# keychera/raytracing-clj

Measured on AMD Instinct MI355X. Metric: Mray-samples/sec at 1200×675×100spp depth50; achieved HBM GB/s vs peak, higher is better.
Workload: dtype fp32

## Files before the change

raytracing-clj_amd/csrc/trace.hip:

```cpp
#include "trace_kernel.h"
#include "first_hit.h"
#include "bvh_refit.h"
#include "dscene.h"

namespace rtclj {

__device__ __forceinline__ int cost_bucket(unsigned c) {
  if (c < 8) return static_cast<int>(c);
  const int e = 31 - __clz(c);
  return ((e - 2) << 3) | static_cast<int>((c >> (e - 3)) & 7u);
}
__global__ __launch_bounds__(1024) void order_kernel(unsigned* __restrict__ cost, int* __restrict__ order,
                                                     int n) {
  __shared__ int hist[256];
  __shared__ int cursor[256];
  __shared__ int scan[256];
  const int t = static_cast<int>(threadIdx.x);
  if (t < 256) hist[t] = 0;
  __syncthreads();
  for (int i = t; i < n; i += 1024) atomicAdd(&hist[cost_bucket(cost[i])], 1);
  __syncthreads();
  if (t < 256) scan[t] = hist[255 - t];
  __syncthreads();
  for (int off = 1; off < 256; off <<= 1) {
// ... 115 lines not shown
  for (int p = p0; p < p1; ++p) sum += fin(p);
  __syncthreads();
  s_part[tid] = sum;
  __syncthreads();
  if (tid == 0) {
    int run = 0;
    for (int i = 0; i < 1024; ++i) {
      const int v = s_part[i];
      s_part[i] = run;
      run += v;
    }
    s_left = run;
  }
  __syncthreads();
  int base = s_part[tid];
  for (int p = p0; p < p1; ++p) {
    const int sp = fin(p);
    const int tile = order[p];
    for (int k = 0; k < sp; ++k) units[base + k] = make_int2(tile, k | (sp << 8));
    base += sp;
  }
  for (int u = s_left + tid; u < U; u += 1024) units[u] = make_int2(-1, 0);
}

#ifdef RTCLJ_DIAG
constexpr bool kDiag = true;
#else
constexpr bool kDiag = false;
#endif
static_assert(policy::kTile == kTile && policy::kPoolPx == kPoolPx && policy::kXBytes == kXBytes,
              "variant_policy.h: the kernels' shapes");
constexpr bool traits_agree() {
  for (const policy::Traits& t : policy::kTraits) {
    if (t.build == policy::BUILD_NONE) continue;
    const int walk = t.scan == SCAN_BVHS ? policy::WALK_SORTED : is_bvh_scan(t.scan) ? policy::WALK_BVH : policy::WALK_NONE;
    if (t.walk != walk || t.tree != scan_tree(t.scan) || t.compact != is_compact_scan(t.scan) ||
        t.entry_bytes != stack_entry_bytes(t.scan) || policy::variant_rows(t) != (t.th ? t.th : tile_rows(t.scan)) ||
        (walk == policy::WALK_SORTED && t.threads != kSortThreads))
      return false;
  }
  return true;
}
static_assert(traits_agree(), "variant_policy.h: a row's columns against its scan's traits");

const void* trace_kernel_w16();
static const policy::Traits& variant_traits(int v) { return policy::traits(v, kDiag); }
static const void* variant_fn(int v) {
  switch (v) {
    case policy::kDefault: return RT_K(SRC_LDS, SCAN_BVHQ, false);
    case policy::kScan: return RT_K(SRC_SCALAR, SCAN_GROUP4, false);
    case policy::kGlobal: return RT_K(SRC_SCALAR, SCAN_BVH, false);
    case policy::kFull4: return RT_K(SRC_LDS, SCAN_BVHQ, false);
    case policy::kLeaf8: return RT_KW(SRC_LDS, SCAN_BVHO, false, 8);
    case policy::kCompact: return RT_K(SRC_LDS, SCAN_BVHQ7, false);
    case policy::kCompactW8: return RT_KW(SRC_LDS, SCAN_BVHQ7, false, 8);
    case policy::kCompactW16: return trace_kernel_w16();
    case policy::kCompactTh4: return RT_KWT(SRC_LDS, SCAN_BVHQ7, false, 4, 4);
  }
#ifdef RTCLJ_DIAG
  return diag_kernel(v);
#else
  return nullptr;
#endif
}
static const void* variant_sweep(int v) { return v == policy::kCompact ? RT_KSW(SRC_LDS, SCAN_BVHQ7, 4, 0) : nullptr; }

static std::atomic<int> g_variant{0};
static std::atomic<int> g_schedule{0};
static const bool g_bvh_sah = bvh_sah_default();
#ifdef RTCLJ_DIAG
static const bool g_timeline = [] {
  const char* e = std::getenv("RTCLJ_TIMELINE");
  return e && std::atoi(e) != 0;
}();
#endif
constexpr int kDbg = 32;
constexpr int kDbgDevices = 64;
static std::mutex g_dbg_mu;
static unsigned long long* g_dbg[kDbgDevices] = {};
static unsigned long long* g_dbgw[kDbgDevices] = {};

int selected_variant() { return g_variant.load(); }
bool diag_build() { return kDiag; }

}

using namespace rtclj;

hipError_t rtclj::fill_words(void* p, uint32_t word, size_t n, hipStream_t stream) {
  if (n == 0) return hipSuccess;
  const size_t blocks = std::min<size_t>((n + 255) / 256, 2048);
  return enqueue(fill_kernel, dim3(static_cast<unsigned>(blocks)), dim3(256), 0, stream, static_cast<uint32_t*>(p), word, n);
}

namespace rtclj {
int fill_async(void* p, int byte_value, size_t bytes, void* stream) {
  if (bytes % 4 != 0) return hipErrorInvalidValue;
  return fill_words(p, static_cast<uint32_t>(byte_value & 0xff) * 0x01010101u, bytes / 4, static_cast<hipStream_t>(stream));
}

int quantize_launch(const float* d_lin, uint8_t* d_out, size_t n, void* stream) {
  if (n == 0) return hipSuccess;
  const size_t blocks = std::min<size_t>((n + 255) / 256, 4096);
  return enqueue(quantize_kernel, dim3(static_cast<unsigned>(blocks)), dim3(256), 0, static_cast<hipStream_t>(stream), d_lin,
                 d_out, n, quantize_table());
}
}

static std::atomic<uint64_t> g_scene_uid{0};
uint64_t rtclj::scene_uid(const rt_dscene* ds) { return ds ? ds->uid : 0; }
// ... 738 lines not shown
```

raytracing-clj_amd/csrc/trace_kernel.h:

```cpp
#pragma once
#include <hip/hip_runtime.h>

#include <algorithm>
#include <chrono>
#include <atomic>
#include <climits>
#include <cstdlib>
#include <cmath>
#include <cstdint>
#include <cstring>
#include <mutex>
#include <string>
#include <thread>
#include <type_traits>
#include <vector>

#include "bvh.h"
#include "bvh_pad.h"
#include "fp_rn.h"
#include "rt_internal.h"

namespace rtclj {

struct alignas(16) KArgs {
  const float4* geo;
  const struct Pair* geo2;
  const float4* sph;
  const float4* mat;
  const int* kind;
  float* out;
  unsigned long long* counters;
  unsigned long long* dbg;
  unsigned long long* dbgw;
  float cam[18];
  int defocus;
  int n;
  int n_pad;
  int width;
  int rows_out;
  int row_begin, row_tile, tile_first, tile_step;
  const float4* bvh_blob;
  int bvh_blob_f4;
  int bvh_off_pairs;
  int bvh_off_pidx;
  int big_pair0;
  int n_big_leaves;
  int bvh_stack;
  float bvh_c[3], bvh_r;
  float bvh_c0;
  const int* tile_order;
  unsigned* tile_cost;
  unsigned long long* part;
  int tiles_x;
  int n_whole, split;
  const int2* unit_tab;
  uint64_t rt_magic;
  int spp, sample_begin, max_depth;
  int realm;
  int sampler;
  uint32_t key;
  unsigned long long* word;
  unsigned* done;
  unsigned long long* sum;
  int* owner;
  unsigned long long* stealc;
  int n_owner;
  int n_units;
  int share_from;
  int steal_min;
  int batch_max;
  int lds_batch_max;
  unsigned epoch;
  int compact;
// ... 158 lines not shown
  asm volatile("" : "+s"(p));
  return p;
}

enum { SRC_LDS = 1, SRC_SCALAR = 2 };
enum { SCAN_SIMPLE = 0, SCAN_GROUP4 = 1, SCAN_PK4 = 2, SCAN_BVH = 3, SCAN_BVHWW = 4, SCAN_BVHQ = 5, SCAN_BVHO = 6,
       SCAN_BVHS = 7 ,
       SCAN_BVHQ7 = 8  };
constexpr bool is_bvh_scan(int scan) { return (scan >= SCAN_BVH && scan <= SCAN_BVHO) || scan == SCAN_BVHQ7; }
constexpr bool is_q(int scan) { return scan == SCAN_BVHQ || scan == SCAN_BVHQ7; }
constexpr int leaf_pairs(int scan) { return scan == SCAN_BVHO ? 4 : is_q(scan) ? 2 : 1; }
constexpr int scan_tree(int scan) { return scan == SCAN_BVHO ? 2 : (is_q(scan) || scan == SCAN_BVHS) ? 1 : 0; }
constexpr bool is_compact_scan(int scan) { return scan == SCAN_BVHQ7; }
constexpr int stack_entry_bytes(int scan) { return (scan == SCAN_BVHO || scan == SCAN_BVHQ7) ? 1 : 2; }

typedef float f2 __attribute__((ext_vector_type(2)));
typedef const char __attribute__((address_space(3)))* LdsC;
typedef const f2 __attribute__((address_space(3)))* LdsF2;
typedef float f4v __attribute__((ext_vector_type(4)));
typedef const f4v __attribute__((address_space(3)))* LdsF4;
typedef const long long __attribute__((address_space(3)))* LdsI64;
__device__ __forceinline__ unsigned lds_addr(const void* p) { return static_cast<unsigned>((uintptr_t)(LdsC)p); }
struct alignas(16) Pair {
  f2 x, y, z, w;
};
__device__ __forceinline__ f2 fma2(f2 a, f2 b, f2 c) { return __builtin_elementwise_fma(a, b, c); }
__device__ __forceinline__ float fma3(float a, float b, float c) {
  float r;
  asm("v_fma_f32 %0, %1, %2, %3" : "=v"(r) : "v"(a), "v"(b), "v"(c));
  return r;
}
__device__ __forceinline__ f2 bc_lo(f2 v) { return __builtin_shufflevector(v, v, 0, 0); }
__device__ __forceinline__ f2 bc_hi(f2 v) { return __builtin_shufflevector(v, v, 1, 1); }

struct alignas(16) KNode {
  f2 x[3], y[3], z[3];
  int c0, c1;
};
static_assert(sizeof(KNode) == 80, "KNode layout");

constexpr int kTile = 8;
constexpr int kLeafRecBytes = 80;
constexpr int kPoolPx = kTile * kTile;
constexpr int tile_rows(int scan) { return scan == SCAN_BVHS ? 16 : kTile; }

constexpr int min_waves(int scan, bool stats, int nw = 4) {
  return stats ? 1 : scan == SCAN_BVHQ ? 6 : scan == SCAN_BVHQ7 ? (nw == 16 ? 8 : 7) : scan == SCAN_BVHO ? 3 : 1;
}

template <int SRC, int SCAN, class F>
__device__ void diag_scan(const struct KArgs& a, const float4* s_geo, float ox, float oy, float oz, float ux,
                          float uy, float uz, F&& consider);

template <int SRC, int SCAN, bool STATS = false, int NW = 4, int THT = 0, bool SWEEP = false>
__global__ __launch_bounds__(64 * NW, min_waves(SCAN, STATS, NW)) void trace_kernel(const KArgs a) {
  constexpr int NT = 64 * NW;
  __shared__ int s_pool_next;
  __shared__ int s_cnt;
  __shared__ int s_join;
  __shared__ int s_unit[2];
  __shared__ unsigned long long s_best;
  __shared__ unsigned long long s_segs;
  __shared__ int s_last;
  __shared__ int s_mb_post[NW], s_mb_take[NW], s_alive, s_mb_avail;
  __shared__ int s_mb_lim[NW];
  constexpr int TH = THT ? THT : tile_rows(SCAN);
  constexpr int NPX = kTile * TH;
  using AccT = std::conditional_t<SCAN == SCAN_BVHQ7, unsigned, unsigned long long>;
  __shared__ AccT s_acc[NPX * 3];
  uint64_t st_iter = 0, st_lanes = 0, st_sph = 0, st_blk = 0, st_blk_lanes = 0;
  uint64_t st_trav = 0, st_trav_lanes = 0;
  uint64_t st_leafw = 0, st_consw = 0;
  uint64_t st_ball = 0, st_disk = 0;
  uint64_t st_fl = 0;
  uint64_t st_fresh = 0, st_fresh_lanes = 0;
  uint64_t st_diel = 0, st_diel_lanes = 0;
  uint64_t st_lm = 0, st_lm_lanes = 0;
  uint64_t st_sums = 0, st_refill = 0, st_claim = 0, st_drain = 0;
  uint64_t st_c_cam = 0, st_c_scan = 0, st_c_shade = 0, st_c_acc = 0, st_ts = 0;
  uint64_t st_t0 = 0;
  if (STATS || a.tile_cost || a.dbgw) st_t0 = __builtin_amdgcn_s_memrealtime();
  extern __shared__ __attribute__((aligned(16))) float4 s_geo[];
  const int n = a.n;
  const int lane = threadIdx.x & 63;
  const int unit = static_cast<int>(blockIdx.x);
  const KArgsP ka = kargs_opaque();
  const bool own = SWEEP || unit < ka->n_units;
  int xpool = 0;
  if constexpr (SWEEP) {
    xpool = static_cast<int>(__hip_atomic_load(&ka->xq_n[0], __ATOMIC_RELAXED, __HIP_MEMORY_SCOPE_AGENT));
    if (unit * NT >= xpool) return;
  }
  auto tile_pool = [&](KArgsP kp, int t) {
    const int ty = t / kp->tiles_x, tx = t - ty * kp->tiles_x;
    const int w = max(0, min(kTile, kp->width - tx * kTile)), h = max(0, min(TH, kp->rows_out - ty * TH));
    return kp->spp > 0 && kp->max_depth > 0 ? w * h * kp->spp : 0;
  };
  if (!own) {
    if (!ka->word) return;
    if (threadIdx.x == 0) {
      s_best = 0ull;
      s_unit[0] = -1;
    }
    __syncthreads();
    const int M = ka->n_owner;
    const int w0 = static_cast<int>(mix32(static_cast<uint32_t>(unit)) % static_cast<uint32_t>(M));
    unsigned long long key = 0;
// ... 120 lines not shown
  };
  const float cx = a.cam[0], cy = a.cam[1], cz = a.cam[2];

  const int k0 = split ? static_cast<int>(static_cast<int64_t>(split_ix) * ka->spp / nsplit) : 0;
  const int cnt = split ? static_cast<int>(static_cast<int64_t>(split_ix + 1) * ka->spp / nsplit) - k0 : ka->spp;
  const int pool = SWEEP ? xpool : (cnt > 0 && ka->max_depth > 0) ? npx * cnt : 0;
  const uint32_t mag_vw = vw > 0 ? 0xffffffffu / static_cast<uint32_t>(vw) + 1u : 0u;
  const uint32_t mag16_vw = vw > 0 ? (65536u + static_cast<uint32_t>(vw) - 1u) / static_cast<uint32_t>(vw) : 0u;
  const uint64_t npx_magic = npx > 1 ? ~0ull / static_cast<uint64_t>(npx) + 1ull : 0ull;
  const bool shared_tile = !SWEEP && ka->word && !split && (!own || (pool > 512 && unit >= ka->share_from));
  unsigned long long* const src = shared_tile ? ka->word + tile : nullptr;
  const int kc_batch_max = ka->batch_max > 0 ? ka->batch_max : min(1024, max(kShareBatch, (pool / 48) & ~63));
  if (threadIdx.x == 0) {
    if (own && shared_tile) {
      __hip_atomic_exchange(&ka->word[tile], (static_cast<unsigned long long>(ka->epoch) << 48) | static_cast<unsigned long long>(NT),
                            __ATOMIC_RELAXED, __HIP_MEMORY_SCOPE_AGENT);
      __hip_atomic_exchange(&ka->owner[unit % ka->n_owner], tile, __ATOMIC_RELAXED, __HIP_MEMORY_SCOPE_AGENT);
      s_cnt = NT;
    }
    s_join = own ? 0 : 1;
    s_segs = 0ull;
    s_pool_next = NT;
    s_alive = NW;
    s_mb_avail = 0;
  }
  if (threadIdx.x < NW) {
    s_mb_post[threadIdx.x] = 0;
    s_mb_take[threadIdx.x] = 0;
    s_mb_lim[threadIdx.x] = ka->compact > 0 ? ka->compact : -1;
  }
  if (threadIdx.x < NPX * 3) s_acc[threadIdx.x] = 0;
  constexpr bool kPixelTable = is_q(SCAN) && !SWEEP;
  constexpr bool kCompactPx = SCAN == SCAN_BVHQ7;
  __shared__ std::conditional_t<kCompactPx, uint32_t, float4> s_px[kPixelTable ? NPX : 1];
  __shared__ float s_prow[kCompactPx ? TH : 1];
  if constexpr (kPixelTable) {
    const int t = static_cast<int>(threadIdx.x);
    if (t < npx) {
      const int qy = vw == 1 ? t : static_cast<int>(__umulhi(static_cast<uint32_t>(t), mag_vw));
      const int px = qx0 + (t - qy * vw);
      const int gy = image_row(qy0 + qy);
      if constexpr (kCompactPx) {
        s_px[t] = pixel_key(px, gy);
        if (px == qx0) s_prow[qy] = static_cast<float>(gy);
      } else {
        s_px[t] = make_float4(__uint_as_float(pixel_key(px, gy)), static_cast<float>(px), static_cast<float>(gy), 0.0f);
      }
    }
  }
  __shared__ uint32_t s_carry[kCompactPx ? NPX * 3 / 4 : 1];
  if constexpr (kCompactPx) {
    if (threadIdx.x < NPX * 3 / 4) s_carry[threadIdx.x] = 0u;
  }
  __syncthreads();
  int wb = 0, we = 0;
  int j = first + static_cast<int>(threadIdx.x), q = 0, k = 0;
  bool active = j < pool;
  if (!active) j = -2;

  uint32_t st = 0;
  float ox = 0, oy = 0, oz = 0, dx = 0, dy = 0, dz = 0;
  float tr = 1, tg = 1, tb = 1;
  int rem = 0;
  int last = -1;
  bool fresh = true;


  constexpr bool kCompact = is_bvh_scan(SCAN);
  const int wv = static_cast<int>(threadIdx.x >> 6);
  auto mb_word = [&](int d, int f, int p, int P) -> uint32_t* {
    constexpr int SZ = static_cast<int>(sizeof(StackT));
    constexpr int W = 16 * SZ;
    const int i = f * P + p;
    return reinterpret_cast<uint32_t*>(reinterpret_cast<char*>(s_stack) + (i / W) * NT * SZ + d * 64 * SZ +
                                       (i % W) * 4);
  };
  auto lds_load = [](int* p) { return __hip_atomic_load(p, __ATOMIC_ACQUIRE, __HIP_MEMORY_SCOPE_WORKGROUP); };
  auto compact_step = [&]() {
    RT_MARK("compact_step");
    const int wu = static_cast<int>(__builtin_amdgcn_readfirstlane(threadIdx.x >> 6));
    const int P = kargs_opaque()->mb_paths;
    const int leader = static_cast<int>(__builtin_amdgcn_readfirstlane(lane));
    const uint64_t live = __ballot(active);
    const int left = static_cast<int>(__popcll(live));
    bool out = false;
    bool post = false;
    if constexpr (!SWEEP) {
      uint4* const xq = kargs_opaque()->xq;
      if (xq) {
        if (left > 0) {
          int base = 0;
          if (lane == leader) base = static_cast<int>(atomicAdd(&kargs_opaque()->xq_n[0], static_cast<unsigned>(left)));
          base = __builtin_amdgcn_readlane(base, leader);
          const int rank = static_cast<int>(__builtin_amdgcn_mbcnt_hi(static_cast<uint32_t>(live >> 32),
                                                                      __builtin_amdgcn_mbcnt_lo(static_cast<uint32_t>(live), 0u)));
          if (active) {
            const int qy = static_cast<int>(__umul24(static_cast<uint32_t>(q), mag16_vw) >> 16);
            const int pix = (qy0 + qy) * kargs_opaque()->width + qx0 + (q - qy * vw);
            uint4* r = xq + 4 * static_cast<size_t>(base + rank);
            r[0] = make_uint4(__float_as_uint(ox), __float_as_uint(oy), __float_as_uint(oz), __float_as_uint(dx));
            r[1] = make_uint4(__float_as_uint(dy), __float_as_uint(dz), __float_as_uint(tr), __float_as_uint(tg));
            r[2] = make_uint4(__float_as_uint(tb), st, static_cast<uint32_t>(pix), static_cast<uint32_t>(rem));
            reinterpret_cast<uint32_t*>(r + 3)[0] = static_cast<uint32_t>(last);
          }
        }
        if (lane == leader) atomicAdd(&s_alive, -1);
        active = false;
// ... 36 lines not shown
          __hip_atomic_store(&s_mb_post[wu], 0, __ATOMIC_RELAXED, __HIP_MEMORY_SCOPE_WORKGROUP);
          atomicAdd(&s_mb_avail, -left);
        }
      }
      old = __builtin_amdgcn_readlane(old, leader);
      if (old > 1) {
        active = false;
        j = -2;
        return;
      }
      out = true;
    }
    uint64_t freem = ~live;
    bool took = false;
#pragma unroll 1
    for (int d = 0; d < NW && freem; ++d) {
      if (d == wu) continue;
      const int posted = sgpr(lds_load(&s_mb_post[d]));
      if (posted <= sgpr(lds_load(&s_mb_take[d]))) continue;
      const int want = static_cast<int>(__popcll(freem));
      int t0 = 0;
      if (lane == leader) t0 = atomicAdd(&s_mb_take[d], want);
      t0 = __builtin_amdgcn_readlane(t0, leader);
      const int got = min(want, posted - t0);
      if (got <= 0) continue;
      if (lane == leader) atomicAdd(&s_mb_avail, -got);
      const int rank = static_cast<int>(__builtin_amdgcn_mbcnt_hi(static_cast<uint32_t>(freem >> 32),
                                                                  __builtin_amdgcn_mbcnt_lo(static_cast<uint32_t>(freem), 0u)));
      const bool mine = ((freem >> lane) & 1ull) && rank < got;
      if (mine) {
        const int p = t0 + rank;
        ox = __uint_as_float(*mb_word(d, 0, p, P));
        oy = __uint_as_float(*mb_word(d, 1, p, P));
        oz = __uint_as_float(*mb_word(d, 2, p, P));
        dx = __uint_as_float(*mb_word(d, 3, p, P));
        dy = __uint_as_float(*mb_word(d, 4, p, P));
        dz = __uint_as_float(*mb_word(d, 5, p, P));
        tr = __uint_as_float(*mb_word(d, 6, p, P));
        tg = __uint_as_float(*mb_word(d, 7, p, P));
        tb = __uint_as_float(*mb_word(d, 8, p, P));
        st = *mb_word(d, 9, p, P);
        q = static_cast<int>(*mb_word(d, 10, p, P));
        rem = static_cast<int>(*mb_word(d, 11, p, P));
        last = static_cast<int>(*mb_word(d, 12, p, P));
        active = true;
        fresh = false;
        j = -1;
      }
      freem &= ~__ballot(mine);
      took = true;
    }
    if (out && (took || left > 0) && lane == leader) atomicAdd(&s_alive, 1);
  };
  auto iteration = [&]() {
    bool done = false;
    if constexpr (STATS) st_ts = stamp();
    if constexpr (STATS) {
      const uint64_t ex = __builtin_amdgcn_read_exec();
      if (lane == __ffsll(static_cast<long long>(ex)) - 1) {
        ++st_iter;
        st_lanes += __popcll(ex);
      }
    }
    RT_MARK("iteration");
    if (kCompact ? j >= 0 : fresh) {
      RT_MARK("camera");
      if constexpr (SWEEP) {
        const uint4* r = kargs_opaque()->xq + 4 * static_cast<size_t>(j);
        const uint4 r0 = r[0], r1 = r[1], r2 = r[2];
        const uint32_t r3 = reinterpret_cast<const uint32_t*>(r + 3)[0];
        ox = __uint_as_float(r0.x);
        oy = __uint_as_float(r0.y);
        oz = __uint_as_float(r0.z);
        dx = __uint_as_float(r0.w);
        dy = __uint_as_float(r1.x);
        dz = __uint_as_float(r1.y);
        tr = __uint_as_float(r1.z);
        tg = __uint_as_float(r1.w);
        tb = __uint_as_float(r2.x);
        st = r2.y;
        q = static_cast<int>(r2.z);
        rem = static_cast<int>(r2.w);
        last = static_cast<int>(r3);
        fresh = false;
        j = -1;
      } else {
      if constexpr (STATS) {
        const uint64_t ex = __builtin_amdgcn_read_exec();
        if (lane == __ffsll(static_cast<long long>(ex)) - 1) {
          ++st_fresh;
          st_fresh_lanes += __popcll(ex);
        }
      }
      k = div_magic(j, npx_magic);
      q = j - k * npx;
      uint32_t pk;
      float fpx, fgy;
      if constexpr (kPixelTable && kCompactPx) {
        pk = s_px[q];
        const int qy = static_cast<int>(__umul24(static_cast<uint32_t>(q), mag16_vw) >> 16);
        fpx = static_cast<float>(qx0 + (q - qy * vw));
        fgy = s_prow[qy];
      } else if constexpr (kPixelTable) {
        const float4 pt = s_px[q];
        pk = __float_as_uint(pt.x);
        fpx = pt.y;
        fgy = pt.z;
      } else {
        const int qy = vw == 1 ? q : static_cast<int>(__umulhi(static_cast<uint32_t>(q), mag_vw));
        const int px = qx0 + (q - qy * vw);
        const int gy = image_row(qy0 + qy);
        pk = pixel_key(px, gy);
        fpx = static_cast<float>(px);
        fgy = static_cast<float>(gy);
      }
      st = mix32(pk + static_cast<uint32_t>(a.sample_begin + k0 + k) * 0x9e3779b9u);
// ... 206 lines not shown
          if constexpr (STATS) {
            const uint64_t ex = __builtin_amdgcn_read_exec();
            if (lane == __ffsll(static_cast<long long>(ex)) - 1) ++st_consw;
          }
          const unsigned k = __builtin_ctz(m);
          m &= m - 1;
          float h = hh[0], d = dd[0];
          int s = ii[0];
#pragma unroll
          for (int j = 1; j < 2 * NP; ++j) {
            h = k == static_cast<unsigned>(8 * j) ? hh[j] : h;
            d = k == static_cast<unsigned>(8 * j) ? dd[j] : d;
            s = k == static_cast<unsigned>(8 * j) ? ii[j] : s;
          }
          consider_tie(h, d, s);
        }
        }
      };
      auto node_planes = [&](int node, float& tn0, float& tn1, float& tf0, float& tf1, int& c0, int& c1) {
        if constexpr (STATS) st_fl += 24;
        const unsigned nof = SCAN == SCAN_BVHQ    ? static_cast<unsigned>(node)
                             : SCAN == SCAN_BVHQ7 ? __umul24(static_cast<unsigned>(node), 80u) + lds_addr(nodes)
                                                  : __umul24(static_cast<unsigned>(node), 80u);
        f2 x0, x1, y0, y1, z0, z1;
        int2 ch;
        if constexpr (SRC == SRC_LDS && is_q(SCAN)) {
          const LdsF2 lx = (LdsF2)(uintptr_t)(nof + offx), ly = (LdsF2)(uintptr_t)(nof + offy),
                      lz = (LdsF2)(uintptr_t)(nof + offz);
          x0 = lx[0], x1 = lx[1], y0 = ly[0], y1 = ly[1], z0 = lz[0], z1 = lz[1];
          const long long c2 = *(LdsI64)(uintptr_t)(nof + 72);
          ch = make_int2(static_cast<int>(c2), static_cast<int>(c2 >> 32));
        } else {
          const char* nb = reinterpret_cast<const char*>(nodes) + nof;
          const f2* ax = reinterpret_cast<const f2*>(nb + offx);
          const f2* ay = reinterpret_cast<const f2*>(nb + offy);
          const f2* az = reinterpret_cast<const f2*>(nb + offz);
          x0 = ax[0], x1 = ax[1], y0 = ay[0], y1 = ay[1], z0 = az[0], z1 = az[1];
          ch = *reinterpret_cast<const int2*>(nb + 72);
        }
        asm volatile("" : "+v"(r_x), "+v"(r_y), "+v"(r_z), "+v"(nf_x), "+v"(nf_y), "+v"(nf_z));
        const PadAxis px = {r_x.x, r_x.y, nf_x.x, nf_x.y, 0}, py = {r_y.x, r_y.y, nf_y.x, nf_y.y, 0},
                      pz = {r_z.x, r_z.y, nf_z.x, nf_z.y, 0};
        pad_interval(px, py, pz, x0.x, x1.x, y0.x, y1.x, z0.x, z1.x, tn0, tf0);
        pad_interval(px, py, pz, x0.y, x1.y, y0.y, y1.y, z0.y, z1.y, tn1, tf1);
        c0 = ch.x;
        c1 = ch.y;
      };
      auto node_test = [&](int node, float& tn0, float& tn1, bool& hit0, bool& hit1, int& c0, int& c1) {
        float tf0, tf1;
        node_planes(node, tn0, tn1, tf0, tf1, c0, c1);
        hit0 = pad_meets(tn0, tf0, tmin, best_t);
        hit1 = pad_meets(tn1, tf1, tmin, best_t);
      };
      RT_MARK("bigleaf");
      for (int b = 0; b < a.n_big_leaves; ++b) {
        if constexpr (kLeafRec)
          leaf(static_cast<int>(lds_addr(nodes)) + a.bvh_off_pairs + ((a.big_pair0 >> 1) + b) * kLeafRecBytes);
        else
          leaf(a.big_pair0 + b * leaf_pairs(SCAN));
      }
      RT_MARK("tree_setup");
      int node = SRC == SRC_LDS && SCAN == SCAN_BVHQ ? static_cast<int>(lds_addr(nodes)) : 0;
      unsigned tix = threadIdx.x;
      asm volatile("" : "+v"(tix));
      StackT* top = s_stack + tix;
      int row_b = NT * static_cast<int>(sizeof(StackT));
      asm volatile("" : "+v"(row_b));
      bool go = true;
      while (go) {
        RT_MARK("node");
        if constexpr (STATS) {
          ++st_sph;
          const uint64_t ex = __builtin_amdgcn_read_exec();
          if (lane == __ffsll(static_cast<long long>(ex)) - 1) {
            ++st_trav;
            st_trav_lanes += __popcll(ex);
          }
        }
        float tn0, tn1;
        bool hit0, hit1;
        int c0, c1;
        node_test(node, tn0, tn1, hit0, hit1, c0, c1);
        const bool l0 = hit0 && c0 < 0, l1 = hit1 && c1 < 0;
        if (l0 || l1) {
          leaf(l0 ? ~c0 : ~c1);
          if (l0 && l1) leaf(~c1);
        }
        const bool i0 = hit0 && !l0, i1 = hit1 && !l1;
        const bool sw = tn1 < tn0;
        int nxt = (i0 && (!i1 || !sw)) ? c0 : c1;
        *top = static_cast<StackT>(sw ? c0 : c1);
        top = reinterpret_cast<StackT*>(reinterpret_cast<char*>(top) + ((i0 && i1) ? row_b : 0));
        if (!(i0 || i1)) {
          top -= NT;
          go = top >= s_stack;
          nxt = *top;
        }
        node = nxt;
      }
      RT_MARK("hit");
      ox = o_xy.x;
      oy = o_xy.y;
      oz = o_zux.x;
      ux = o_zux.y;
      uy = u_yz.x;
      uz = u_yz.y;
    } else {
      auto load = [&](int s) -> float4 {
        if constexpr (SRC == SRC_LDS) return s_geo[s];
        else return a.geo[s];
      };
      float4 g0 = load(0), g1 = load(1), g2 = load(2), g3 = load(3);
      for (int s = 0; s < n; s += 4) {
        const float4 n0 = load(s + 4), n1 = load(s + 5), n2 = load(s + 6), n3 = load(s + 7);
        float h[4], disc[4];
        bool cand[4];
#pragma unroll
        for (int k = 0; k < 4; ++k) {
          const float4 g = k == 0 ? g0 : k == 1 ? g1 : k == 2 ? g2 : g3;
          const float ocx = g.x - ox, ocy = g.y - oy, ocz = g.z - oz;
          h[k] = fmaf(uz, ocz, fmaf(uy, ocy, ux * ocx));
          const float c = fmaf(ocx, ocx, fmaf(ocz, ocz, fmaf(ocy, ocy, g.w)));
          disc[k] = fmaf(h[k], h[k], -c);
          cand[k] = fminf(disc[k], fmaxf(h[k], -c)) >= 0.0f;
        }
        if (cand[0] | cand[1] | cand[2] | cand[3]) {
#pragma unroll
          for (int k = 0; k < 4; ++k)
            if (cand[k]) consider(h[k], disc[k], s + k);
        }
        g0 = n0;
        g1 = n1;
        g2 = n2;
        g3 = n3;
      }
    }
    if constexpr (STATS && !is_bvh_scan(SCAN)) st_fl += 16ull * static_cast<uint64_t>(n);
    if constexpr (STATS && !is_bvh_scan(SCAN)) {
      const uint64_t ex = __builtin_amdgcn_read_exec();
      if (lane == __ffsll(static_cast<long long>(ex)) - 1) st_sph += static_cast<uint64_t>(n);
    }

    if constexpr (STATS) {
      const uint64_t t = stamp();
      st_c_scan += t - st_ts;
      st_ts = t;
    }
    float cr = 0.0f, cg = 0.0f, cb = 0.0f;
    if (best < 0) {
      if constexpr (STATS) st_fl += 12;
      const float sa = 0.5f * (uy + 1.0f);
// ... 97 lines not shown
        }
        if constexpr (STATS) st_fl += refl ? 7 : 22;
        if (refl) {
          const float k2 = 2.0f * un;
          dx = fmaf(-nx, k2, ux);
          dy = fmaf(-ny, k2, uy);
          dz = fmaf(-nz, k2, uz);
        } else {
          const float qx = fmaf(nx, cosv, ux) * ri;
          const float qy = fmaf(ny, cosv, uy) * ri;
          const float qz = fmaf(nz, cosv, uz) * ri;
          const float par = -sqrt_rn(fabsf(1.0f - fmaf(qz, qz, fmaf(qy, qy, qx * qx))));
          dx = fmaf(nx, par, qx);
          dy = fmaf(ny, par, qy);
          dz = fmaf(nz, par, qz);
        }
      }
    }

    if constexpr (STATS) {
      const uint64_t t = stamp();
      st_c_shade += t - st_ts;
      st_ts = t;
    }
    RT_MARK("sums");
    if (done) {
      if constexpr (STATS) st_fl += 3;
      if constexpr (STATS) wave_event(st_sums);
      AccT* acc = &s_acc[q * 3];
      if constexpr (SWEEP) {
        unsigned long long* pp = kargs_opaque()->part + static_cast<size_t>(q) * 3;
        const uint32_t f0 = fix24(cr), f1 = fix24(cg), f2 = fix24(cb);
        if (f0) __hip_atomic_fetch_add(pp + 0, static_cast<unsigned long long>(f0), __ATOMIC_RELAXED, __HIP_MEMORY_SCOPE_AGENT);
        if (f1) __hip_atomic_fetch_add(pp + 1, static_cast<unsigned long long>(f1), __ATOMIC_RELAXED, __HIP_MEMORY_SCOPE_AGENT);
        if (f2) __hip_atomic_fetch_add(pp + 2, static_cast<unsigned long long>(f2), __ATOMIC_RELAXED, __HIP_MEMORY_SCOPE_AGENT);
      } else if (kCompactPx && sgpr(kargs_opaque()->spp) > 255) {
        const uint32_t f0 = fix24(cr), f1 = fix24(cg), f2 = fix24(cb);
        const uint32_t o0 = __hip_atomic_fetch_add(acc + 0, f0, __ATOMIC_RELAXED, __HIP_MEMORY_SCOPE_WORKGROUP);
        const uint32_t o1 = __hip_atomic_fetch_add(acc + 1, f1, __ATOMIC_RELAXED, __HIP_MEMORY_SCOPE_WORKGROUP);
        const uint32_t o2 = __hip_atomic_fetch_add(acc + 2, f2, __ATOMIC_RELAXED, __HIP_MEMORY_SCOPE_WORKGROUP);
        const bool w0 = o0 + f0 < o0, w1 = o1 + f1 < o1, w2 = o2 + f2 < o2;
        if (w0 | w1 | w2) {
          RT_MARK("cold");
          const int c = q * 3;
          if (w0) atomicAdd(&s_carry[c >> 2], 1u << (8 * (c & 3)));
          if (w1) atomicAdd(&s_carry[(c + 1) >> 2], 1u << (8 * ((c + 1) & 3)));
          if (w2) atomicAdd(&s_carry[(c + 2) >> 2], 1u << (8 * ((c + 2) & 3)));
        }
      } else {
        __hip_atomic_fetch_add(acc + 0, static_cast<AccT>(fix24(cr)), __ATOMIC_RELAXED, __HIP_MEMORY_SCOPE_WORKGROUP);
        __hip_atomic_fetch_add(acc + 1, static_cast<AccT>(fix24(cg)), __ATOMIC_RELAXED, __HIP_MEMORY_SCOPE_WORKGROUP);
        __hip_atomic_fetch_add(acc + 2, static_cast<AccT>(fix24(cb)), __ATOMIC_RELAXED, __HIP_MEMORY_SCOPE_WORKGROUP);
      }
    }
    RT_MARK("refill");
    const uint64_t m = __ballot(done);
    if (m) {
      if constexpr (STATS) wave_event(st_refill);
      const int need = static_cast<int>(__popcll(m));
      const int rank = static_cast<int>(__builtin_amdgcn_mbcnt_hi(static_cast<uint32_t>(m >> 32),
                                                                  __builtin_amdgcn_mbcnt_lo(static_cast<uint32_t>(m), 0u)));
      int nj = -1;
      for (int r0 = 0;;) {
        const int take = min(we - wb, need - r0);
        if (rank >= r0 && rank < r0 + take) nj = wb + (rank - r0);
        wb += take;
        r0 += take;
        if (r0 >= need || we >= pool) break;
        RT_MARK("claim");
        if constexpr (STATS) wave_event(st_claim);
        int g = 0;
        const int want = src ? max(kShareBatch, min(kc_batch_max, ((pool - we) >> 3) & ~63))
                             : max(64, min(kargs_opaque()->lds_batch_max, ((pool - we) >> 3) & ~63));
        const int leader = static_cast<int>(__builtin_amdgcn_readfirstlane(lane));
        if (lane == leader) {
          if (src) {
            const unsigned long long wd = __hip_atomic_fetch_add(src, static_cast<unsigned long long>(want),
                                                                 __ATOMIC_RELAXED, __HIP_MEMORY_SCOPE_AGENT);
            g = static_cast<int>(static_cast<unsigned>(wd));
            if (g < pool) atomicAdd(&s_cnt, min(pool - g, want));
            atomicMax(&s_join, word_helpers(wd));
          } else if constexpr (SWEEP) {
            g = static_cast<int>(atomicAdd(&kargs_opaque()->xq_n[1], 64u)) + static_cast<int>(gridDim.x) * NT;
          } else {
            g = atomicAdd(&s_pool_next, want);
          }
        }
        g = __builtin_amdgcn_readlane(g, leader);
        wb = min(g, pool);
        we = min(g + (SWEEP ? 64 : want), pool);
        if (wb >= pool) we = pool;
      }
      RT_MARK("refill");
      if (done) {
        j = kCompact && nj < 0 ? -2 : nj;
        fresh = true;
        if (nj < 0) active = false;
      }
    }
    if constexpr (STATS) st_c_acc += stamp() - st_ts;
    RT_MARK("compaction");
    if constexpr (kCompact) {
      if (wb >= pool) {
        RT_MARK("drain_check");
        if constexpr (STATS) wave_event(st_drain);
        const int lim = sgpr(lds_load(&s_mb_lim[threadIdx.x >> 6]));
        if (lim >= 0) {
          const int left = static_cast<int>(__popcll(__ballot(j >= -1)));
          if ((left <= lim || (left < 64 && sgpr(lds_load(&s_mb_avail)) > 0)) && __ballot(j >= 0) == 0 &&
              j == -1)
            j = -3;
        }
      }
    }
  };
  for (;;) {
    RT_MARK("loop");
    if constexpr (kCompact) {
      while (j >= -1) iteration();
    } else {
      while (active) iteration();
    }
    if constexpr (!kCompact) {
      break;
    } else {
      if (sgpr(lds_load(&s_mb_lim[wv])) < 0) break;
      wb = we = pool;
      active = j == -3;
      if (active) j = -1;
      compact_step();
      if (__ballot(active) == 0) break;
    }
  }

  RT_MARK("epilogue");
  __syncthreads();
  const KArgsP ke = kargs_opaque();
  if constexpr (!SWEEP) {
  const int t = static_cast<int>(threadIdx.x);
  const bool alone = !shared_tile || sgpr(s_join) == 0;
  auto out_index = [&](int tt) {
    const int fp = tt / 3, ch = tt - 3 * fp;
    const int qy = vw == 1 ? fp : static_cast<int>(__umulhi(static_cast<uint32_t>(fp), mag_vw));
    const int px = qx0 + (fp - qy * vw), ro = qy0 + qy;
    return (static_cast<size_t>(ro) * ke->width + px) * 3 + ch;
  };
  auto write_mean = [&](size_t e, unsigned long long sum) {
    const float tot = static_cast<float>(sum) * 0x1p-24f;
    const float inv = static_cast<float>(ke->spp > 0 ? ke->spp : 1);
    ke->out[e] = ke->realm ? tot * (1.0f / inv) : tot / inv;
  };
  auto total = [&](int tt) -> unsigned long long {
    unsigned long long v = static_cast<unsigned long long>(s_acc[tt]);
    if constexpr (kCompactPx) v += static_cast<unsigned long long>((s_carry[tt >> 2] >> (8 * (tt & 3))) & 0xffu) << 32;
    return v;
  };
  if (split) {
    if (t < npx * 3) {
      const unsigned long long v = total(t);
      if (v) __hip_atomic_fetch_add(&ke->part[out_index(t)], v, __ATOMIC_RELAXED, __HIP_MEMORY_SCOPE_AGENT);
    }
  } else if (alone) {
    if (t < npx * 3) write_mean(out_index(t), total(t));
  } else {
    unsigned long long* gs = ke->sum + static_cast<size_t>(tile) * (NPX * 3);
    if (t < npx * 3) {
// ... 122 lines not shown
```

raytracing-clj_amd/csrc/variant_policy.h:

```cpp
#pragma once
#include <algorithm>
#include <cstddef>
#include <cstdint>

#include "bvh.h"

namespace rtclj {
namespace policy {

constexpr int kTile = 8;
constexpr int kPoolPx = kTile * kTile;
constexpr size_t kXBytes = 8 * 11 * 64 * 4;
constexpr int kFeatThreads = 256;
enum { FEAT_LDS = 0, FEAT_GLOBAL = 1, FEAT_SCAN = 2 };

enum : int {
  kDefault = 0,
  kScan = 5,
  kGlobal = 12,
  kFull4 = 16,
  kLeaf8 = 18,
  kCompact = 22,
  kCompactW8 = 24,
  kCompactW16 = 26,
  kCompactTh4 = 28,
  kVariants = 30
};

enum { WALK_NONE = 0 , WALK_BVH = 1, WALK_SORTED = 2  };
enum { BUILD_NONE = 0, BUILD_PRODUCT = 1, BUILD_DIAG = 2  };

struct Traits {
  int scan;
  int threads;
  int th;
  bool lds;
  bool stats;
  int build;
  int walk;
  int tree;
  bool compact;
  int entry_bytes;
  int stats_build;
};
constexpr Traits kNone{0, 256, 0, false, false, BUILD_NONE, WALK_NONE, 0, false, 2, 0};
constexpr Traits kTraits[kVariants] = {
    {5, 256, 0, true, false, BUILD_PRODUCT, WALK_BVH, 1, false, 2, 0},
    {0, 256, 0, true, false, BUILD_DIAG, WALK_NONE, 0, false, 2, 3},
    {0, 256, 0, false, false, BUILD_DIAG, WALK_NONE, 0, false, 2, 0},
    {0, 256, 0, true, true, BUILD_DIAG, WALK_NONE, 0, false, 2, 0},
    {1, 256, 0, true, false, BUILD_DIAG, WALK_NONE, 0, false, 2, 6},
    {1, 256, 0, false, false, BUILD_PRODUCT, WALK_NONE, 0, false, 2, 7},
    {1, 256, 0, true, true, BUILD_DIAG, WALK_NONE, 0, false, 2, 0},
    {1, 256, 0, false, true, BUILD_DIAG, WALK_NONE, 0, false, 2, 0},
    {2, 256, 0, true, false, BUILD_DIAG, WALK_NONE, 0, false, 2, 0},
    {2, 256, 0, false, false, BUILD_DIAG, WALK_NONE, 0, false, 2, 10},
    {2, 256, 0, false, true, BUILD_DIAG, WALK_NONE, 0, false, 2, 0},
    {3, 256, 0, true, false, BUILD_DIAG, WALK_BVH, 0, false, 2, 13},
    {3, 256, 0, false, false, BUILD_PRODUCT, WALK_BVH, 0, false, 2, 0},
    {3, 256, 0, true, true, BUILD_DIAG, WALK_BVH, 0, false, 2, 0},
    kNone,
    kNone,
    {5, 256, 0, true, false, BUILD_PRODUCT, WALK_BVH, 1, false, 2, 17},
    {5, 256, 0, true, true, BUILD_DIAG, WALK_BVH, 1, false, 2, 0},
    {6, 512, 0, true, false, BUILD_PRODUCT, WALK_BVH, 2, false, 1, 19},
    {6, 512, 0, true, true, BUILD_DIAG, WALK_BVH, 2, false, 1, 0},
    {7, 512, 0, true, false, BUILD_DIAG, WALK_SORTED, 1, false, 2, 0},
    {7, 512, 0, true, false, BUILD_DIAG, WALK_SORTED, 1, false, 2, 0},
    {8, 256, 0, true, false, BUILD_PRODUCT, WALK_BVH, 1, true, 1, 0},
    kNone,
    {8, 512, 0, true, false, BUILD_PRODUCT, WALK_BVH, 1, true, 1, 0},
    kNone,
    {8, 1024, 0, true, false, BUILD_PRODUCT, WALK_BVH, 1, true, 1, 0},
    kNone,
    {8, 256, 4, true, false, BUILD_PRODUCT, WALK_BVH, 1, true, 1, 0},
    kNone,
};
constexpr bool has_variant(int v, bool diag) {
  return v >= 0 && v < kVariants && (kTraits[v].build == BUILD_PRODUCT || (diag && kTraits[v].build == BUILD_DIAG));
}
constexpr const Traits& traits(int v, bool diag) { return has_variant(v, diag) ? kTraits[v] : kNone; }
constexpr int variant_rows(const Traits& t) { return t.th ? t.th : t.walk == WALK_SORTED ? 16 : kTile; }

struct Tree {
  int n_nodes, depth, blob_f4;
};
struct Scene {
  Tree tree[3];
  int n_pad;
  bool unit_albedo;
};
struct Frame {
  int width, height, rows, spp;
};

inline int stack_entries(const Tree& t, int tree) { return tree == 0 ? t.depth + 2 : std::max(t.depth, 1); }
inline size_t stack_of(const Tree& t, int tree, int threads = 256) {
  return static_cast<size_t>(stack_entries(t, tree)) * threads * (tree == 2 ? 1 : 2);
}
inline size_t lds_of(const Tree& t, int tree, int threads = 256) {
  return static_cast<size_t>(t.blob_f4) * 16 + stack_of(t, tree, threads);
}
inline int stack_entries_compact(const Tree& t) { return std::max(t.depth, 1); }
inline size_t lds_of_compact(const Tree& t, int threads) {
  return static_cast<size_t>(t.blob_f4) * 16 + static_cast<size_t>(stack_entries_compact(t)) * threads;
}
constexpr size_t kStaticLds = 4 + kPoolPx * 3 * 8 + kPoolPx * 16 + 12;
constexpr size_t kLds5 = 160 * 1024 / 5 - kStaticLds;
constexpr size_t kStaticLds8 = 2048;

inline int resolve_variant(const Scene& ds, int vsel, bool diag) {
  const auto tr = [diag](int v) -> const Traits& { return traits(v, diag); };
  if (vsel == kDefault)
    vsel = (lds_of(ds.tree[1], 1) > kLds5 && ds.tree[2].n_nodes <= 256 &&
            lds_of(ds.tree[2], 2, tr(kLeaf8).threads) < lds_of(ds.tree[1], 1)) ? kLeaf8 : kFull4;
  if (tr(vsel).tree == 2 && ds.tree[2].n_nodes > 256) vsel = tr(vsel).stats ? tr(kFull4).stats_build : kFull4;
  if (tr(vsel).walk == WALK_BVH && tr(vsel).tree == 1 && !tr(vsel).compact && ds.tree[1].n_nodes * 80 + 8192 > 65535)
    vsel = kGlobal;
  if (tr(vsel).walk == WALK_SORTED &&
      (ds.tree[1].n_nodes * 80 > 65535 || ds.tree[1].depth + 2 > kBvhStack ||
       static_cast<size_t>(ds.tree[1].blob_f4) * 16 + kXBytes > 96 * 1024))
    vsel = kFull4;
  if (tr(vsel).walk != WALK_NONE) {
    const int tree = tr(vsel).tree;
    const Tree& t = ds.tree[tree];
    if (t.depth + 2 > kBvhStack) return kScan;
    if (tr(vsel).lds && lds_of(t, tree, tr(vsel).threads) > 96 * 1024)
      vsel = kGlobal;
// ... 77 lines not shown
```

Before: 17540.

## Add per-tile conservative leaf culling list for first-bounce rays in compact kernel

```diff
diff --git a/raytracing-clj_amd/csrc/tile_list.h b/raytracing-clj_amd/csrc/tile_list.h
--- /dev/null
+++ b/raytracing-clj_amd/csrc/tile_list.h
@@ -0,0 +1,66 @@
+#pragma once
+#include <cmath>
+
+#if defined(__HIPCC__)
+#define RT_TL_FN __host__ __device__ __forceinline__
+#else
+#define RT_TL_FN inline
+#endif
+
+namespace rtclj {
+
+constexpr double kTlRel = 2e-3;
+constexpr double kTlAbs = 4e-6;
+
+struct TileRays {
+  double c[3], v[3];
+  double rl, rf;
+  double mabs;
+};
+
+RT_TL_FN TileRays tile_rays(const float* cam, int defocus, float x0, float x1, float y0, float y1, double rf_scale = 1.0) {
+  TileRays t;
+  const double fx = 0.5 * (static_cast<double>(x0) + x1), fy = 0.5 * (static_cast<double>(y0) + y1);
+  const double hx = 0.5 * (static_cast<double>(x1) - x0) + 0.5, hy = 0.5 * (static_cast<double>(y1) - y0) + 0.5;
+  double uu = 0, vv = 0, uv = 0, dudu = 0, dvdv = 0, dudv = 0, nc = 0, nf = 0;
+  for (int k = 0; k < 3; ++k) {
+    const double du = cam[6 + k], dv = cam[9 + k], U = defocus ? cam[12 + k] : 0.0, V = defocus ? cam[15 + k] : 0.0;
+    const double f0 = cam[3 + k] + fx * du + fy * dv;
+    t.c[k] = cam[k];
+    t.v[k] = f0 - t.c[k];
+    uu += U * U, vv += V * V, uv += U * V;
+    dudu += du * du, dvdv += dv * dv, dudv += du * dv;
+    nc += t.c[k] * t.c[k], nf += f0 * f0;
+  }
+  t.rl = sqrt((uu > vv ? uu : vv) + fabs(uv));
+  const double rf = rf_scale * sqrt(hx * hx * dudu + hy * hy * dvdv + 2.0 * hx * hy * fabs(dudv));
+  t.mabs = kTlAbs * (sqrt(nc) + sqrt(nf) + t.rl + rf);
+  t.rf = rf + t.mabs;
+  return t;
+}
+
+RT_TL_FN bool tile_keeps(const TileRays& t, float cx, float cy, float cz, float w) {
+  if (w == INFINITY) return false;
+  const double r = sqrt(-static_cast<double>(w));
+  const double wx = cx - t.c[0], wy = cy - t.c[1], wz = cz - t.c[2];
+  const double ww = wx * wx + wy * wy + wz * wz;
+  const double wv = wx * t.v[0] + wy * t.v[1] + wz * t.v[2];
+  const double vv = t.v[0] * t.v[0] + t.v[1] * t.v[1] + t.v[2] * t.v[2];
+  const double M = sqrt(ww) + t.rl + r, e1 = kTlRel * M, e2 = e1 * e1 / (2.0 * r);
+  const double K = r + (e2 < e1 ? e2 : e1) + t.mabs;
+  auto excluded = [&](double a0, double a1, bool finite) {
+    const double A = vv - a1 * a1, B = wv + a0 * a1, Cq = ww - a0 * a0;
+    const double q1 = A - 2.0 * B + Cq;
+    if (!(q1 > 0.0)) return false;
+    if (finite && !(Cq > 0.0)) return false;
+    if (!(A > 0.0)) return finite && A <= 0.0;
+    const double sv = B / A;
+    const bool inside = finite ? (sv > 0.0 && sv < 1.0) : sv > 1.0;
+    if (!(sv == sv)) return false;
+    if (inside && !(Cq - B * sv > 0.0)) return false;
+    return true;
+  };
+  return !(excluded(K + t.rl, t.rf - t.rl, true) && excluded(K - t.rl, t.rf + t.rl, false));
+}
+
+}
diff --git a/raytracing-clj_amd/csrc/trace.hip b/raytracing-clj_amd/csrc/trace.hip
--- a/raytracing-clj_amd/csrc/trace.hip
+++ b/raytracing-clj_amd/csrc/trace.hip
@@ -191,10 +191,11 @@
     case policy::kGlobal: return RT_K(SRC_SCALAR, SCAN_BVH, false);
     case policy::kFull4: return RT_K(SRC_LDS, SCAN_BVHQ, false);
     case policy::kLeaf8: return RT_KW(SRC_LDS, SCAN_BVHO, false, 8);
-    case policy::kCompact: return RT_K(SRC_LDS, SCAN_BVHQ7, false);
+    case policy::kCompact: return reinterpret_cast<const void*>(&trace_kernel<SRC_LDS, SCAN_BVHQ7, false, 4, 0, false, true>);
     case policy::kCompactW8: return RT_KW(SRC_LDS, SCAN_BVHQ7, false, 8);
     case policy::kCompactW16: return trace_kernel_w16();
     case policy::kCompactTh4: return RT_KWT(SRC_LDS, SCAN_BVHQ7, false, 4, 4);
+    case policy::kCompactWalk: return RT_K(SRC_LDS, SCAN_BVHQ7, false);
   }
 #ifdef RTCLJ_DIAG
   return diag_kernel(v);
diff --git a/raytracing-clj_amd/csrc/trace_kernel.h b/raytracing-clj_amd/csrc/trace_kernel.h
--- a/raytracing-clj_amd/csrc/trace_kernel.h
+++ b/raytracing-clj_amd/csrc/trace_kernel.h
@@ -19,6 +19,7 @@
 #include "bvh_pad.h"
 #include "fp_rn.h"
 #include "rt_internal.h"
+#include "tile_list.h"
 
 namespace rtclj {
 
@@ -283,7 +284,7 @@
 __device__ void diag_scan(const struct KArgs& a, const float4* s_geo, float ox, float oy, float oz, float ux,
                           float uy, float uz, F&& consider);
 
-template <int SRC, int SCAN, bool STATS = false, int NW = 4, int THT = 0, bool SWEEP = false>
+template <int SRC, int SCAN, bool STATS = false, int NW = 4, int THT = 0, bool SWEEP = false, bool PRE = false>
 __global__ __launch_bounds__(64 * NW, min_waves(SCAN, STATS, NW)) void trace_kernel(const KArgs a) {
   constexpr int NT = 64 * NW;
   __shared__ int s_pool_next;
@@ -510,7 +511,38 @@
   if constexpr (kCompactPx) {
     if (threadIdx.x < NPX * 3 / 4) s_carry[threadIdx.x] = 0u;
   }
+  constexpr int kTlMax = 14;
+  unsigned* s_tl = nullptr;
+  if constexpr (PRE) {
+    __shared__ unsigned tl_words[8];
+    s_tl = tl_words;
+    if (threadIdx.x == 0) tl_words[0] = 0u;
+  }
   __syncthreads();
+  if constexpr (PRE) {
+    static_assert(SRC == SRC_LDS && is_q(SCAN) && !SWEEP, "the tile list: the 4-body tree's leaf records in LDS");
+    if (npx > 0) {
+      const TileRays tr = tile_rays(a.cam, a.defocus, static_cast<float>(qx0), static_cast<float>(qx0 + vw - 1),
+                                    static_cast<float>(image_row(qy0)), static_cast<float>(image_row(qy0 + vh - 1)));
+      const int n_rec = (a.bvh_off_pidx - a.bvh_off_pairs) >> 6;
+      const unsigned rec0 = lds_addr(s_geo) + static_cast<unsigned>(a.bvh_off_pairs >> 4) * 16u;
+      for (int i = static_cast<int>(threadIdx.x); i < n_rec; i += NT) {
+        const unsigned ra = rec0 + static_cast<unsigned>(i) * kLeafRecBytes;
+        bool any = false;
+#pragma unroll 1
+        for (unsigned b = 0; b < 4; ++b) {
+          const f4v g = *(LdsF4)(uintptr_t)(ra + 16u * b);
+          any = any || tile_keeps(tr, g.x, g.y, g.z, g.w);
+        }
+        if (any) {
+          const unsigned slot = atomicAdd(&s_tl[0], ra > 0xffffu ? static_cast<unsigned>(kTlMax + 1) : 1u);
+          if (slot < static_cast<unsigned>(kTlMax))
+            reinterpret_cast<unsigned short*>(s_tl + 1)[slot] = static_cast<unsigned short>(ra);
+        }
+      }
+    }
+    __syncthreads();
+  }
   int wb = 0, we = 0;
   int j = first + static_cast<int>(threadIdx.x), q = 0, k = 0;
   bool active = j < pool;
@@ -653,7 +685,8 @@
     }
     if (out && (took || left > 0) && lane == leader) atomicAdd(&s_alive, 1);
   };
-  auto iteration = [&]() {
+  auto segment = [&](auto list_tag) __attribute__((always_inline)) {
+    constexpr bool LIST = decltype(list_tag)::value;
     bool done = false;
     if constexpr (STATS) st_ts = stamp();
     if constexpr (STATS) {
@@ -663,6 +696,8 @@
         st_lanes += __popcll(ex);
       }
     }
+    const bool in = !PRE || (LIST ? j >= 0 : j >= -1);
+    if (in) {
     RT_MARK("iteration");
     if (kCompact ? j >= 0 : fresh) {
       RT_MARK("camera");
@@ -975,6 +1010,11 @@
         hit0 = pad_meets(tn0, tf0, tmin, best_t);
         hit1 = pad_meets(tn1, tf1, tmin, best_t);
       };
+      if constexpr (LIST) {
+        RT_MARK("tile_list");
+        const int n_list = min(sgpr(static_cast<int>(s_tl[0])), kTlMax);
+        for (int b = 0; b < n_list; ++b) leaf(static_cast<int>(reinterpret_cast<const unsigned short*>(s_tl + 1)[b]));
+      } else {
       RT_MARK("bigleaf");
       for (int b = 0; b < a.n_big_leaves; ++b) {
         if constexpr (kLeafRec)
@@ -1020,6 +1060,7 @@
           nxt = *top;
         }
         node = nxt;
+      }
       }
       RT_MARK("hit");
       ox = o_xy.x;
@@ -1223,6 +1264,7 @@
         __hip_atomic_fetch_add(acc + 1, static_cast<AccT>(fix24(cg)), __ATOMIC_RELAXED, __HIP_MEMORY_SCOPE_WORKGROUP);
         __hip_atomic_fetch_add(acc + 2, static_cast<AccT>(fix24(cb)), __ATOMIC_RELAXED, __HIP_MEMORY_SCOPE_WORKGROUP);
       }
+    }
     }
     RT_MARK("refill");
     const uint64_t m = __ballot(done);
@@ -1271,7 +1313,7 @@
     }
     if constexpr (STATS) st_c_acc += stamp() - st_ts;
     RT_MARK("compaction");
-    if constexpr (kCompact) {
+    if constexpr (kCompact && !LIST) {
       if (wb >= pool) {
         RT_MARK("drain_check");
         if constexpr (STATS) wave_event(st_drain);
@@ -1283,6 +1325,26 @@
             j = -3;
         }
       }
+    }
+  };
+#ifdef RTCLJ_PRE_TRIPS
+  constexpr int kPreTrips = RTCLJ_PRE_TRIPS;
+#else
+  constexpr int kPreTrips = 2;
+#endif
+  auto iteration = [&]() {
+    if constexpr (PRE) {
+      if (sgpr(static_cast<int>(s_tl[0])) <= kTlMax) {
+#pragma unroll 1
+        for (int trip = 0; trip < kPreTrips; ++trip) {
+          if (__ballot(j >= 0) == 0) break;
+          segment(std::true_type{});
+        }
+        if (__ballot(j == -1) == 0) return;
+      }
+      segment(std::false_type{});
+    } else {
+      segment(std::false_type{});
     }
   };
   for (;;) {
diff --git a/raytracing-clj_amd/csrc/variant_policy.h b/raytracing-clj_amd/csrc/variant_policy.h
--- a/raytracing-clj_amd/csrc/variant_policy.h
+++ b/raytracing-clj_amd/csrc/variant_policy.h
@@ -24,7 +24,8 @@
   kCompactW8 = 24,
   kCompactW16 = 26,
   kCompactTh4 = 28,
-  kVariants = 30
+  kCompactWalk = 30,
+  kVariants = 32
 };
 
 enum { WALK_NONE = 0 , WALK_BVH = 1, WALK_SORTED = 2  };
@@ -74,6 +75,8 @@
     {8, 1024, 0, true, false, BUILD_PRODUCT, WALK_BVH, 1, true, 1, 0},
     kNone,
     {8, 256, 4, true, false, BUILD_PRODUCT, WALK_BVH, 1, true, 1, 0},
+    kNone,
+    {8, 256, 0, true, false, BUILD_PRODUCT, WALK_BVH, 1, true, 1, 0},
     kNone,
 };
 constexpr bool has_variant(int v, bool diag) {
```

New measurement: 19170 (median of 6 runs). +9.3%, better.
